# Druthyn/rtiow

Measured on AMD Instinct MI355X. Metric: Msamples/sec (pixels×spp) on book-1 final scene; per-pixel RMSE vs CPU, higher is better.
Workload: dtype f64

## Files before the change

__graft_entry__.py:

```python
import os
import subprocess
import sys

ROOT = os.path.dirname(os.path.abspath(__file__))
if ROOT not in sys.path:
    sys.path.insert(0, ROOT)

HIPCC_FLAGS = [
    "-O3", "-std=c++17", "--offload-arch=gfx950",
    "-ffp-contract=off",
    "-fhip-fp32-correctly-rounded-divide-sqrt",
    "-mllvm", "-amdgpu-mfma-vgpr-form",
    "-fPIC", "-shared",
]


def build_hip_library(crosscheck=False, count_features=False):
    out = os.path.join(ROOT, "tools", "librtiow_hip_xcheck.so") if crosscheck else os.path.join(ROOT, "rtiow_amd", "librtiow_hip.so")
    if count_features:
        out = os.path.join(ROOT, "tools", "lib_features_count.so")
    srcs = [os.path.join(ROOT, "rtiow_amd", "csrc", name) for name in ("rt_api.hip", "rt_frames.hip", "rt_features.hip")]
    import bench
    cmd = ["hipcc", *HIPCC_FLAGS, *(["-DRTIOW_CROSSCHECK_MODES"] if crosscheck else []), *(["-DRT_FEATURES_COUNT"] if count_features else []),
           f'-DRT_SOURCE_SHA="{bench.kernel_source_sha()}"',
           "-I", os.path.join(ROOT, "include"), "-I", os.path.join(ROOT, "rtiow_amd", "csrc"), "-o", out, *srcs]
    subprocess.run(cmd, check=True, cwd=ROOT)
    return out


def build_host_cli(sanitize=False):
    out = os.path.join(ROOT, "host", "rtiow_render_san" if sanitize else "rtiow_render")
    rocm = os.environ.get("ROCM_PATH", "/opt/rocm")
    opt = ["-O1", "-g", "-fno-omit-frame-pointer", "-fsanitize=address,undefined", "-fno-sanitize-recover=all"] if sanitize else ["-O2"]
    cmd = ["g++", *opt, "-std=c++17", "-ffp-contract=off", "-Wall", "-Wextra", "-Wno-unused-parameter",
           "-I", os.path.join(ROOT, "include"), "-I", os.path.join(ROOT, "host"), "-isystem", os.path.join(rocm, "include"),
           "-o", out, os.path.join(ROOT, "host", "rtiow_render.cpp"),
           "-L", os.path.join(ROOT, "rtiow_amd"), "-lrtiow_hip", "-L", os.path.join(rocm, "lib"), "-lamdhip64", "-lrccl",
           "-pthread", "-Wl,-rpath,$ORIGIN/../rtiow_amd", "-Wl,-rpath," + os.path.join(rocm, "lib")]
    subprocess.run(cmd, check=True, cwd=ROOT)
    return out


def build() -> None:
    build_hip_library()
    build_hip_library(crosscheck=True)
    build_host_cli()
    subprocess.run(["make", "-s", "-C", os.path.join(ROOT, "oracle"), "liboracle.so"], check=True)
    import rtiow_amd
    from rtiow_amd import _ffi
    lib = _ffi.load()
    assert lib.rt_backend_name() == b"hip-gfx950"
    assert not _ffi.has_crosscheck_modes()
    assert rtiow_amd.SPHERE_DTYPE.itemsize == 72


def smoke() -> None:
    import numpy as np
    import oracle
    import rtiow_amd as rt

    w, h, spp = 96, 54, 4
    flat = rt.random_scene(1).flatten()
    cam = rt.book1_camera(w, h)
    with rt.Renderer(0) as r:
        r.upload_scene(flat)
        sums, fix, st = r.render(cam, rt.make_params(w, h, spp, seed=1))
        rgba = r.resolve_rgba8(fix, spp, flip=True)
    want_fix, want_sum, ost = oracle.render_b(oracle.camera_from_host(cam), flat, oracle.make_params(w, h, spp, seed=1))
    assert np.array_equal(fix, want_fix), "GPU exact sums differ from the CPU oracle"
    assert np.array_equal(sums, want_sum)
    assert st["rays_traced"] == ost["rays_traced"] and st["samples"] == w * h * spp
    assert np.array_equal(rgba, oracle.resolve_b(want_fix, spp, flip=True))
    with rt.Renderer(0) as r:
        r.upload_scene(flat)
# ... 11 lines not shown
```

rtiow_amd/_ffi.py:

```python
import ctypes as C
import os

_HERE = os.path.dirname(os.path.abspath(__file__))
LIB_PATH = os.environ.get("RTIOW_HIP_LIB") or os.path.join(_HERE, "librtiow_hip.so")


class rt_sphere(C.Structure):
    _fields_ = [("center", C.c_double * 3), ("radius", C.c_double), ("albedo", C.c_double * 3),
                ("param", C.c_double), ("kind", C.c_int32), ("reserved", C.c_int32)]


class rt_camera(C.Structure):
    _fields_ = [("origin", C.c_double * 3), ("lower_left_corner", C.c_double * 3),
                ("horizontal", C.c_double * 3), ("vertical", C.c_double * 3),
                ("u", C.c_double * 3), ("v", C.c_double * 3), ("lens_radius", C.c_double)]


class rt_params(C.Structure):
    _fields_ = [("width", C.c_int32), ("height", C.c_int32), ("spp", C.c_int32),
                ("sample_begin", C.c_int32), ("max_depth", C.c_int32), ("t_min", C.c_double),
                ("seed", C.c_uint64), ("tile_rows", C.c_int32), ("shard_index", C.c_int32),
                ("shard_count", C.c_int32), ("flags", C.c_uint32)]


# ... 13 lines not shown
RT_FLAG_DIAG_STATS = 0x4
RT_FLAG_UNIFORM53 = 0x8
RT_FLAG_OVERLAPPED = 0x10
RT_FLAG_KNOWN = 0x1f
RT_FEATURE_WORDS = 8

_VP = C.c_void_p
SYMBOLS = [
    ("rt_create", C.c_int, [C.c_int32, C.POINTER(_VP)]),
    ("rt_destroy", C.c_int, [_VP]),
    ("rt_upload_scene", C.c_int, [_VP, C.POINTER(rt_sphere), C.c_int32]),
    ("rt_shard_rows", C.c_int, [C.POINTER(rt_params), C.POINTER(C.c_int32)]),
    ("rt_shard_row_index", C.c_int, [C.POINTER(rt_params), C.c_int32, C.POINTER(C.c_int32)]),
    ("rt_render", C.c_int, [_VP, C.POINTER(rt_camera), C.POINTER(rt_params), _VP, _VP, C.POINTER(rt_stats)]),
    ("rt_render_device", C.c_int, [_VP, C.POINTER(rt_camera), C.POINTER(rt_params), _VP, _VP]),
    ("rt_fix_to_f32_device", C.c_int, [_VP, _VP, C.c_int64, _VP, _VP]),
    ("rt_last_stats", C.c_int, [_VP, C.POINTER(rt_stats)]),
    ("rt_resolve_rgba8_device", C.c_int, [_VP, _VP, C.c_int32, C.c_int32, C.c_int64, C.c_int32, _VP, _VP]),
    ("rt_resolve_rgba8", C.c_int, [_VP, _VP, C.c_int32, C.c_int32, C.c_int64, C.c_int32, _VP]),
    ("rt_render_rgba8", C.c_int, [_VP, C.POINTER(rt_camera), C.POINTER(rt_params), C.c_int32, _VP, C.POINTER(rt_stats)]),
    ("rt_render_pixels_device", C.c_int, [_VP, C.POINTER(rt_camera), C.POINTER(rt_params), _VP, C.c_int64, _VP, _VP]),
    ("rt_render_pixels", C.c_int, [_VP, C.POINTER(rt_camera), C.POINTER(rt_params), _VP, C.c_int64, _VP, C.POINTER(rt_stats)]),
    ("rt_select_pixels_device", C.c_int, [_VP, _VP, _VP, _VP, C.c_int32, C.c_int32, C.c_int32, C.POINTER(rt_adaptive), _VP, _VP, _VP]),
    ("rt_select_pixels_host", C.c_int, [_VP, _VP, _VP, C.c_int32, C.c_int32, C.c_int32, C.POINTER(rt_adaptive), _VP, C.POINTER(C.c_int64)]),
    ("rt_render_adaptive", C.c_int, [_VP, C.POINTER(rt_camera), C.POINTER(rt_params), C.POINTER(rt_adaptive), _VP, _VP, _VP, C.POINTER(rt_stats)]),
    ("rt_resolve_rgba8_counts_device", C.c_int, [_VP, _VP, _VP, C.c_int32, C.c_int32, C.c_int32, _VP, _VP]),
    ("rt_resolve_rgba8_counts", C.c_int, [_VP, _VP, _VP, C.c_int32, C.c_int32, C.c_int32, _VP]),
    ("rt_render_frames_device", C.c_int, [_VP, _VP, C.c_int32, C.c_int32, C.POINTER(rt_params), _VP, _VP]),
    ("rt_render_frames", C.c_int, [_VP, _VP, C.c_int32, C.c_int32, C.POINTER(rt_params), _VP, C.POINTER(rt_stats)]),
    ("rt_render_frames_rgba8", C.c_int, [_VP, _VP, C.c_int32, C.c_int32, C.POINTER(rt_params), C.c_int32, _VP, C.POINTER(rt_stats)]),
    ("rt_render_features_device", C.c_int, [_VP, C.POINTER(rt_camera), C.POINTER(rt_params), _VP, _VP, _VP]),
    ("rt_render_features", C.c_int, [_VP, C.POINTER(rt_camera), C.POINTER(rt_params), _VP, _VP, C.POINTER(C.c_float)]),
    ("rt_features_to_f32_device", C.c_int, [_VP, _VP, C.c_int32, C.c_int32, C.c_int64, _VP, _VP]),
    ("rt_features_to_f32", C.c_int, [_VP, _VP, C.c_int32, C.c_int32, C.c_int64, _VP]),
    ("rt_last_error", C.c_char_p, []),
    ("rt_backend_name", C.c_char_p, []),
    ("rt_abi_version", C.c_int32, []),
    ("rt_build_source_sha", C.c_char_p, []),
    ("rt_philox_device", C.c_int, [_VP, C.POINTER(C.c_uint32), C.POINTER(C.c_uint32), C.POINTER(C.c_uint32)]),
    ("rt_f64_div_sqrt_device", C.c_int, [_VP, _VP, _VP, C.c_int32, _VP, _VP]),
    ("rt_quantize_device", C.c_int, [_VP, _VP, C.c_int32, _VP]),
    ("rt_unit_accept_device", C.c_int, [_VP, _VP, C.c_int32, _VP, _VP]),
    ("rt_tube_tile_host", C.c_int, [C.POINTER(rt_sphere), _VP, _VP, C.POINTER(C.c_float)]),
    ("rt_tile_layout_host", C.c_int, [C.POINTER(rt_sphere), C.c_int32, C.POINTER(C.c_int32), C.POINTER(C.c_float), C.POINTER(C.c_int32), C.c_int32]),
    ("rt_filter_tube_device", C.c_int, [_VP, _VP, _VP, C.POINTER(rt_sphere), _VP, _VP, _VP, C.POINTER(C.c_float)]),
]

XCHECK_SYMBOLS = [
    ("rt_filter_products_device", C.c_int, [_VP, _VP, _VP, _VP, C.c_int32, _VP, _VP]),
    ("rt_filter_lifted_device", C.c_int, [_VP, _VP, _VP, C.POINTER(rt_sphere), _VP, _VP, _VP]),
    ("rt_grid_cells_device", C.c_int, [_VP, _VP, _VP, C.c_int32, C.POINTER(C.c_float), C.c_int32, C.c_float, _VP, _VP]),
]

_lib = None


class RtiowHipError(RuntimeError):
    pass


def load():
    global _lib
    if _lib is not None:
        return _lib
    if not os.path.exists(LIB_PATH):
        raise RtiowHipError(
            f"{LIB_PATH} not found: build it with ./build_lib.sh (hipcc --offload-arch=gfx950); "
            "there is no CPU fallback for the render path")
    try:
        import torch
    except ImportError:
        pass
    lib = C.CDLL(LIB_PATH)
    for name, res, args in SYMBOLS:
        fn = getattr(lib, name)
        fn.restype = res
        fn.argtypes = args
    for name, res, args in XCHECK_SYMBOLS:
        if hasattr(lib, name):
            fn = getattr(lib, name)
            fn.restype = res
            fn.argtypes = args
    _lib = lib
    return lib


def has_crosscheck_modes():
    return hasattr(load(), "rt_filter_lifted_device")


def check(rc, what):
    if rc != 0:
        msg = load().rt_last_error().decode("utf-8", "replace")
        raise RtiowHipError(f"{what} failed ({rc}): {msg}")
```

rtiow_amd/csrc/rt_api.hip:

```cpp
#include <hip/hip_runtime.h>

#include <algorithm>
#include <cmath>
#include <cstdarg>
#include <cstdio>
#include <cstdlib>
#include <cstring>
#include <vector>

#include "rt_host.hpp"

namespace {

thread_local char g_err[512] = "";

int env_int(const char *name, int dflt)
{
    const char *v = getenv(name);
    if (!v || !*v) return dflt;
    return atoi(v);
}

}

// ... 586 lines not shown
    const bool large_blocks = mode_now == 5 && !(p->flags & RT_FLAG_DIAG_STATS) && use_ring && small_block == (unsigned)rt::kItemBlock &&
                              p->spp >= (small_grid_scene ? rt::kLargeMinSppSmallGrid : rt::kLargeMinSpp) && total_items >= lb_min;
    const unsigned item_block = large_blocks ? rt::kItemBlockLarge : use_ring ? small_block : rt::kItemBlock;
    const unsigned long long n_blocks = (total_items + item_block - 1) / item_block;
    if (n_blocks > 0x7fffffffULL)
        return fail(RT_ERR_INVALID_ARGUMENT, "rows*width*spp = %llu pixel-samples in one launch: at most 2^31 blocks of %d "
                    "(split the samples over several launches with sample_begin and RT_FLAG_ACCUMULATE)", total_items, (int)item_block);
    rt::KParams kp;
    memset(&kp, 0, sizeof(kp));
    static_assert(sizeof(rt::KCamera) == sizeof(rt_camera), "camera layouts must match");
    memcpy(&kp.cam, cam, sizeof(rt_camera));
    kp.width = p->width; kp.height = p->height;
    kp.spp = p->spp; kp.sample_begin = p->sample_begin; kp.max_depth = p->max_depth;
    kp.t_min = p->t_min;
    kp.k0 = (uint32_t)p->seed; kp.k1 = (uint32_t)(p->seed >> 32);
    kp.tile_rows = p->tile_rows; kp.shard_index = p->shard_index; kp.shard_count = p->shard_count;
    kp.rows = rows; kp.n_spheres = ctx->n_spheres;
    kp.npix = (uint32_t)npix; kp.total_items = total_items; kp.n_blocks = (uint32_t)n_blocks;
    kp.inv_spp = p->spp > 0 ? 1.0 / (double)p->spp : 0.0;
    kp.inv_width = 1.0 / (double)p->width;
    auto magic_for = [](long long d) -> uint32_t {
        return (d <= 1 || d >= 32768) ? 0u : (uint32_t)(0x100000000ULL / (unsigned long long)d + 1ULL);
    };
    kp.magic_spp = magic_for(p->spp); kp.magic_width = magic_for(p->width); kp.magic_tile = magic_for(p->tile_rows);
    kp.use_ring = use_ring ? 1 : 0;
    kp.block_items = item_block;
    set_scene_params(ctx, kp);
    kp.fix = (unsigned long long *)d_fix;
    rc = next_launch_slot(ctx, stream, kp);
    if (rc) return rc;

    if (!(p->flags & RT_FLAG_ACCUMULATE) && npix > 0)
        RT_HIP(hipMemsetAsync(d_fix, 0, (size_t)npix * 3 * sizeof(unsigned long long), stream));
    RT_HIP(hipMemsetAsync(ctx->d_queue, 0, 64, stream));
    RT_HIP(hipMemsetAsync(ctx->d_stats, 0, 1024, stream));

    memset(&ctx->last, 0, sizeof(ctx->last));
    ctx->last.n_spheres = ctx->n_spheres;
    ctx->last.block_threads = rt::kBlock;
    ctx->zero_depth_samples = 0;
    if (p->max_depth == 0 || kp.total_items == 0) {
        RT_HIP(hipEventRecord(ctx->ev0, stream));
        RT_HIP(hipEventRecord(ctx->ev1, stream));
        ctx->zero_depth_samples = (unsigned long long)npix * (unsigned long long)p->spp;
        ctx->launched = true;
        return RT_OK;
    }

    int grid = 0;
    const bool diag = (p->flags & RT_FLAG_DIAG_STATS) != 0;
    const int mode = (p->flags & RT_FLAG_NO_FILTER) ? 0 : ctx->scan_mode;
    ctx->last.scan_mode = mode;
    ctx->last.kernel_variant = 0;
    const bool small_grid = small_grid_scene;
    if (p->flags & RT_FLAG_UNIFORM53) {
        if (diag || (mode != 0 && mode != 5))
            return fail(RT_ERR_INVALID_ARGUMENT, "RT_FLAG_UNIFORM53 runs with scan mode 5 (the default) or RT_FLAG_NO_FILTER, without RT_FLAG_DIAG_STATS");
        if (mode == 0) rc = launch_render<0, false, false, true>(ctx, kp, stream, &grid);
        else if (small_grid) rc = large_blocks ? launch_render<5, false, true, true, rt::kItemBlockLarge>(ctx, kp, stream, &grid)
                                              : launch_render<5, false, true, true>(ctx, kp, stream, &grid);
        else rc = large_blocks ? launch_render<5, false, false, true, rt::kItemBlockLarge>(ctx, kp, stream, &grid)
                               : launch_render<5, false, false, true>(ctx, kp, stream, &grid);
        if (rc) return rc;
        ctx->last.kernel_variant = 2 | ((mode == 5 && small_grid) ? 1 : 0) | (mode == 5 && large_blocks ? 4 : 0);
        ctx->launched = true;
        ctx->last.grid_blocks = grid;
        return RT_OK;
    }
    switch (mode * 2 + (diag ? 1 : 0)) {
    case 0: rc = launch_render<0, false>(ctx, kp, stream, &grid); break;
    case 1: rc = launch_render<0, true>(ctx, kp, stream, &grid); break;
    case 2: rc = launch_render<1, false>(ctx, kp, stream, &grid); break;
    case 3: rc = launch_render<1, true>(ctx, kp, stream, &grid); break;
#ifdef RTIOW_CROSSCHECK_MODES
    case 4: rc = launch_render<2, false>(ctx, kp, stream, &grid); break;
    case 5: rc = launch_render<2, true>(ctx, kp, stream, &grid); break;
    case 6: rc = launch_render<3, false>(ctx, kp, stream, &grid); break;
    case 7: rc = launch_render<3, true>(ctx, kp, stream, &grid); break;
    case 8: rc = launch_render<4, false>(ctx, kp, stream, &grid); break;
    case 9: rc = launch_render<4, true>(ctx, kp, stream, &grid); break;
#endif
    case 10:
        if (small_grid) {
            rc = large_blocks ? launch_render<5, false, true, false, rt::kItemBlockLarge>(ctx, kp, stream, &grid)
                              : launch_render<5, false, true>(ctx, kp, stream, &grid);
            ctx->last.kernel_variant = 1;
        } else rc = large_blocks ? launch_render<5, false, false, false, rt::kItemBlockLarge>(ctx, kp, stream, &grid)
                                 : launch_render<5, false>(ctx, kp, stream, &grid);
        if (large_blocks) ctx->last.kernel_variant |= 4;
        break;
    default: rc = launch_render<5, true>(ctx, kp, stream, &grid); break;
    }
    if (rc) return rc;
    ctx->launched = true;
    ctx->last.grid_blocks = grid;
    return RT_OK;
}

int rt_last_stats(rt_context *ctx, rt_stats *stats)
{
    if (!ctx || !stats) return fail(RT_ERR_INVALID_ARGUMENT, "ctx/stats is NULL");
    if (!ctx->launched) return fail(RT_ERR_INVALID_ARGUMENT, "no launch to report on");
    RT_HIP(hipSetDevice(ctx->device));
    RT_HIP(hipEventSynchronize(ctx->ev1));
    float ms = 0.0f;
    RT_HIP(hipEventElapsedTime(&ms, ctx->ev0, ctx->ev1));
    unsigned long long h[80];
    RT_HIP(hipMemcpy(h, ctx->d_stats, sizeof(h), hipMemcpyDeviceToHost));
    for (int k = 0; k < 64; ++k) ctx->last.live_per_bounce[k] = h[16 + k];
    ctx->last.rays_traced = h[0];
    ctx->last.samples = h[1] + ctx->zero_depth_samples;
    ctx->last.candidates = h[2];
    ctx->last.exact_roots = h[3];
    ctx->last.direct_samples = h[4];
    ctx->last.sphere_tests = h[0] * (unsigned long long)(ctx->last.n_spheres > 0 ? ctx->last.n_spheres : 0);
    ctx->last.kernel_ms = ms;
    *stats = ctx->last;
    return RT_OK;
}

#if defined(RT_PHASE_STAMPS) || defined(RT_BLOCK_COUNTS) || defined(RT_EXIT_TIMES) || defined(RT_LDS_CONFLICTS)
extern "C" int rt_debug_phase_cycles(rt_context *ctx, unsigned long long out[8])
{
    RT_HIP(hipSetDevice(ctx->device));
    RT_HIP(hipEventSynchronize(ctx->ev1));
    RT_HIP(hipMemcpy(out, ctx->d_stats + 8, 64, hipMemcpyDeviceToHost));
    return RT_OK;
}
extern "C" int rt_debug_phase_cycles16(rt_context *ctx, unsigned long long out[16])
{
    RT_HIP(hipSetDevice(ctx->device));
    RT_HIP(hipEventSynchronize(ctx->ev1));
    RT_HIP(hipMemcpy(out, ctx->d_stats + 8, 64, hipMemcpyDeviceToHost));
    RT_HIP(hipMemcpy(out + 8, ctx->d_stats + 80, 64, hipMemcpyDeviceToHost));
    return RT_OK;
// ... 545 lines not shown
```

rtiow_amd/csrc/rt_diag.hpp:

```cpp
#pragma once
#include <hip/hip_runtime.h>
#include <stdint.h>

#if (defined(RT_PHASE_STAMPS) + defined(RT_BLOCK_COUNTS) + defined(RT_EXIT_TIMES) + defined(RT_LDS_CONFLICTS)) > 1
#error "one diagnostic build at a time: RT_PHASE_STAMPS, RT_BLOCK_COUNTS, RT_EXIT_TIMES or RT_LDS_CONFLICTS"
#endif

#define RT_DIAG_NOTHING do { } while (0)

#define RT_DIAG_DECLARE() RT_DIAG_NOTHING
#define RT_DIAG_FLUSH() RT_DIAG_NOTHING
#define RT_STAMP(k) RT_DIAG_NOTHING
#define RT_COUNT(k) RT_DIAG_NOTHING
#define RT_COUNT_N(k, n) RT_DIAG_NOTHING
#define RT_COUNT_MAIN(k) RT_DIAG_NOTHING
#define RT_COUNT_ROWS_TRIP(k) RT_DIAG_NOTHING
#define RT_COUNT_ENUM_TRIP(m) RT_DIAG_NOTHING
#define RT_COUNT_REDRAW_LANES(ok) RT_DIAG_NOTHING
#define RT_LDS(site, BYTES, ATOMIC, LOAD64, ptr, active) RT_DIAG_NOTHING
#define RT_LDS_N(site, n, BYTES, ATOMIC, LOAD64, byte_addr, active) RT_DIAG_NOTHING
#define RT_LDS_QUEUE_READS(take, entry) RT_DIAG_NOTHING
#define RT_LDS_POOL_TIE(has_root, r, key) RT_DIAG_NOTHING
#define RT_LDS_ENUM_READS(has, word, summary, seg0) RT_DIAG_NOTHING
#define RT_LDS_RING_ADDS(ringed, my_blk) RT_DIAG_NOTHING

#if defined(RT_PHASE_STAMPS)
#undef RT_DIAG_DECLARE
#undef RT_DIAG_FLUSH
#undef RT_STAMP
#define RT_DIAG_DECLARE() unsigned long long ph[16] = {0, 0, 0, 0, 0, 0, 0, 0, 0, 0, 0, 0, 0, 0, 0, 0}, tprev = __builtin_amdgcn_s_memtime()
#define RT_STAMP(k) do { __builtin_amdgcn_s_waitcnt(0); const unsigned long long tn_ = __builtin_amdgcn_s_memtime(); \
                         __builtin_amdgcn_s_waitcnt(0); ph[k] += tn_ - tprev; tprev = tn_; } while (0)
#define RT_DIAG_FLUSH() do { if (lane == 0) { \
        for (int k_ = 0; k_ < 8; ++k_) atomicAdd(P.stats + 8 + k_, ph[k_]); \
        for (int k_ = 8; k_ < 16; ++k_) atomicAdd(P.stats + 80 + (k_ - 8), ph[k_]); } } while (0)
#endif

#if defined(RT_EXIT_TIMES)
#undef RT_DIAG_DECLARE
#undef RT_DIAG_FLUSH
#define RT_DIAG_DECLARE() const unsigned long long t_wave_start = __builtin_amdgcn_s_memrealtime()
#define RT_DIAG_FLUSH() do { if (lane == 0) { \
        const unsigned long long te_ = __builtin_amdgcn_s_memrealtime(); \
        atomicMax(P.stats + 8, te_); atomicMax(P.stats + 9, ~te_); atomicAdd(P.stats + 10, te_); \
        atomicMax(P.stats + 11, ~t_wave_start); atomicAdd(P.stats + 12, 1ull); } } while (0)
#endif

#if defined(RT_BLOCK_COUNTS)
#undef RT_DIAG_DECLARE
#undef RT_DIAG_FLUSH
#undef RT_COUNT
#undef RT_COUNT_N
#define RT_DIAG_DECLARE() __shared__ unsigned int s_cnt[kBlock / 64][8]; if ((tid & 63) < 8) s_cnt[tid >> 6][tid & 7] = 0u
#define RT_COUNT(k) do { if ((int)(tid & 63) == (int)__builtin_ctzll(__ballot(true))) s_cnt[tid >> 6][k] += 1u; } while (0)
#define RT_COUNT_N(k, n) do { if ((int)(tid & 63) == (int)__builtin_ctzll(__ballot(true))) s_cnt[tid >> 6][k] += (unsigned)(n); } while (0)
#define RT_DIAG_FLUSH() do { if (lane == 0) for (int k_ = 0; k_ < 8; ++k_) atomicAdd(P.stats + 8 + k_, (unsigned long long)s_cnt[tid >> 6][k_]); } while (0)
#if defined(RT_COUNT_ROWS)
#undef RT_COUNT_ROWS_TRIP
#define RT_COUNT_ROWS_TRIP(k) RT_COUNT(k)
#elif defined(RT_COUNT_ENUM)
#undef RT_COUNT_ENUM_TRIP
#define RT_COUNT_ENUM_TRIP(m) do { RT_COUNT(1); RT_COUNT_N(6, __popcll(m)); } while (0)
#elif defined(RT_COUNT_REDRAW)
#undef RT_COUNT_REDRAW_LANES
#define RT_COUNT_REDRAW_LANES(ok) do { const unsigned n1_ = (unsigned)__popcll(__ballot(true)), n6_ = (unsigned)__popcll(__ballot(!(ok))); \
                                       RT_COUNT_N(1, n1_); RT_COUNT_N(6, n6_); } while (0)
#else
#undef RT_COUNT_MAIN
#define RT_COUNT_MAIN(k) RT_COUNT(k)
#endif
#endif

#if defined(RT_LDS_CONFLICTS)
namespace rt {
template <int BYTES, bool ATOMIC, bool LOAD64 = false>
__device__ __noinline__ uint32_t lds_extra_cycles(uint32_t byte_addr, bool active)
{
    constexpr int G = (BYTES == 8 && !LOAD64) ? 16 : 32;
    const int lane = threadIdx.x & 63;
    const unsigned long long m = __ballot(active);
    const uint32_t unit = byte_addr / (uint32_t)BYTES;
    const uint32_t bank = unit % (uint32_t)G;
    bool first = active;
    for (int k = 0; k < 64; ++k) {
        const uint32_t uk = (uint32_t)__builtin_amdgcn_readlane((int)unit, k);
        if (((m >> k) & 1ull) && k < lane && k / G == lane / G && uk == unit) first = false;
    }
    const unsigned long long counted = ATOMIC ? m : __ballot(first);
    uint32_t cnt = 0;
    for (int k = 0; k < 64; ++k) {
        const uint32_t bk = (uint32_t)__builtin_amdgcn_readlane((int)bank, k);
        if (((counted >> k) & 1ull) && k / G == lane / G && bk == bank) cnt++;
    }
    if (!active) cnt = 0;
    uint32_t extra = 0;
    for (int g = 0; g < 64 / G; ++g) {
        uint32_t mx = 0;
        for (int k = g * G; k < (g + 1) * G; ++k) mx = max(mx, (uint32_t)__builtin_amdgcn_readlane((int)cnt, k));
        extra += mx > 1u ? mx - 1u : 0u;
    }
    return extra;
}
}
#undef RT_DIAG_DECLARE
#undef RT_DIAG_FLUSH
#undef RT_LDS
#undef RT_LDS_N
#undef RT_LDS_QUEUE_READS
#undef RT_LDS_POOL_TIE
#undef RT_LDS_ENUM_READS
#undef RT_LDS_RING_ADDS
#define RT_DIAG_DECLARE() unsigned long long lds_x[8] = {0, 0, 0, 0, 0, 0, 0, 0}
#define RT_DIAG_FLUSH() do { if (lane == 0) for (int k_ = 0; k_ < 8; ++k_) atomicAdd(P.stats + 8 + k_, lds_x[k_]); } while (0)
#define RT_LDS(site, BYTES, ATOMIC, LOAD64, ptr, active) do { lds_x[site] += rt::lds_extra_cycles<BYTES, ATOMIC, LOAD64>( \
        (uint32_t)(uintptr_t)(const void __attribute__((address_space(3))) *)(ptr), (active)); } while (0)
#define RT_LDS_N(site, n, BYTES, ATOMIC, LOAD64, byte_addr, active) do { lds_x[site] += (unsigned long long)(n) * \
        rt::lds_extra_cycles<BYTES, ATOMIC, LOAD64>((uint32_t)(byte_addr), (active)); } while (0)
#define RT_LDS_QUEUE_READS(take, entry) do { const bool take_ = (take); const uint32_t e_ = take_ ? (entry) : 0u; \
        RT_LDS(6, 8, false, true, &quv_w[e_], take_); RT_LDS(6, 8, false, true, &quv_w[64 + e_], take_); \
// ... 12 lines not shown
```

rtiow_amd/csrc/rt_host.hpp:

```cpp
#pragma once
#include <hip/hip_runtime.h>

#include "rtiow_hip.h"
#include "rt_kernels.hpp"
#ifdef RTIOW_CROSSCHECK_MODES
#include "xcheck/rt_xcheck_host_ctx.hpp"
#endif

namespace rt_host {
int fail(int code, const char *fmt, ...);
}

#define RT_HIP(call)                                                                          \
    do {                                                                                      \
        hipError_t e_ = (call);                                                               \
        if (e_ != hipSuccess)                                                                 \
            return rt_host::fail(e_ == hipErrorOutOfMemory ? RT_ERR_OUT_OF_MEMORY : RT_ERR_HIP,        \
                        "%s failed: %s (%s:%d)", #call, hipGetErrorString(e_), __FILE__, __LINE__); \
    } while (0)

struct rt_context {
    int device = 0;
    int cu_count = 0;
    float *d_filt = nullptr;
    double *d_geo = nullptr;
    double *d_mat = nullptr;
    uint4 *d_btube = nullptr;
    float tube_rho = 1.0f;
    double *d_geo_slot = nullptr;
    uint32_t *d_slot_orig = nullptr;
    int n_global = 0;
    int grid_dim = 0;
    float grid[8] = {};
    float scene_scale = 0.0f;
#ifdef RTIOW_CROSSCHECK_MODES
    XcheckScene x;
#endif
    int n_tiles = 0;
    int n_always = 0;
    int always_idx[8] = {0, 0, 0, 0, 0, 0, 0, 0};
    int scan_mode = 5;
    int n_spheres = -1;
    static constexpr int kSlots = 2;
    unsigned int *q_slots[kSlots] = {nullptr, nullptr};
    unsigned long long *s_slots[kSlots] = {nullptr, nullptr};
    hipEvent_t e0_slots[kSlots] = {nullptr, nullptr}, e1_slots[kSlots] = {nullptr, nullptr};
    bool slot_used[kSlots] = {false, false};
    int cur = 0;
    unsigned int *d_queue = nullptr;
    unsigned long long *d_stats = nullptr;
    hipEvent_t ev0 = nullptr, ev1 = nullptr;
    hipStream_t own_stream = nullptr;
    bool launched = false;
    unsigned long long zero_depth_samples = 0;
    rt_stats last{};
    void *d_stage_fix = nullptr; size_t stage_fix_bytes = 0;
    void *d_stage_sum = nullptr; size_t stage_sum_bytes = 0;
    void *d_stage_rgba = nullptr; size_t stage_rgba_bytes = 0;
    int blocks_per_cu = 0;
    void *d_sel = nullptr; size_t sel_bytes = 0;
    void *d_adapt = nullptr; size_t adapt_bytes = 0;
    void *d_stage_list = nullptr; size_t stage_list_bytes = 0;
    void *d_stage_cams = nullptr; size_t stage_cams_bytes = 0;
    int ring_min_spp = 0;
};

namespace rt_host {

int validate_params(const rt_params *p);
int ensure(void **ptr, size_t *have, size_t need);
void set_scene_params(const rt_context *ctx, rt::KParams &kp);
int next_launch_slot(rt_context *ctx, hipStream_t stream, rt::KParams &kp);

template <int MODE, bool DIAG, bool SMALLGRID = false, bool U53 = false, int ITEMS = rt::kItemBlock>
int launch_render(rt_context *ctx, const rt::KParams &kp, hipStream_t stream, int *grid_out)
{
    int per_cu = ctx->blocks_per_cu;
    if (per_cu <= 0) {
        int occ = 0;
        RT_HIP(hipOccupancyMaxActiveBlocksPerMultiprocessor(&occ, rt::render_kernel<MODE, DIAG, SMALLGRID, U53, ITEMS>, rt::kBlock, 0));
        per_cu = occ < 1 ? 1 : (occ > 8 ? 8 : occ);
    }
    long long grid = (long long)ctx->cu_count * per_cu;
    const long long need = (long long)((kp.total_items + rt::kBlock - 1) / rt::kBlock);
    if (grid > need) grid = need;
    if (grid < 1) grid = 1;
    *grid_out = (int)grid;
    RT_HIP(hipEventRecord(ctx->ev0, stream));
    hipLaunchKernelGGL((rt::render_kernel<MODE, DIAG, SMALLGRID, U53, ITEMS>), dim3((unsigned)grid), dim3(rt::kBlock), 0, stream, kp);
    RT_HIP(hipGetLastError());
    RT_HIP(hipEventRecord(ctx->ev1, stream));
    return RT_OK;
}

}
```

rtiow_amd/csrc/rt_kernels.hpp:

```cpp
#pragma once
#include "rt_device.hpp"
#include "rt_diag.hpp"
#ifdef RTIOW_CROSSCHECK_MODES
#include "xcheck/rt_xcheck_params.hpp"
#endif
#include <type_traits>

#ifndef RT_GROUP_SKIP
#define RT_GROUP_SKIP 1
#endif

namespace rt {

struct KCamera {
    double origin[3], llc[3], horizontal[3], vertical[3], u[3], v[3];
    double lens_radius;
};

struct KParams {
    KCamera cam;
    double t_min;
    int32_t width, height;
    int32_t spp, sample_begin, max_depth;
    uint32_t k0, k1;
    int32_t tile_rows, shard_index, shard_count;
    int32_t rows;
    int32_t n_spheres;
    int32_t use_ring;
    uint32_t npix;
    uint32_t n_blocks;
    unsigned long long total_items;
    double inv_spp;
    double inv_width;
    uint32_t magic_spp, magic_width, magic_tile;
    uint32_t block_items;
    const float *filt;
#ifdef RTIOW_CROSSCHECK_MODES
    KXcheckTables x;
#endif
    const uint4 *btube;
    float tube_rho;
    float scene_scale;
    const double *geo_slot;
    const uint32_t *slot_orig;
    float grid[8];
    int32_t grid_dim;
    unsigned long long grid_rows;
    int32_t n_global;
    int32_t n_tiles;
    int32_t n_always;
    int32_t always_idx[8];
    const double *geo;
    const double *mat;
    unsigned long long *fix;
    unsigned int *queue;
    unsigned long long *stats;
    const uint32_t *pix_list;
    const KCamera *cams;
    unsigned long long frame_items;
    double inv_frame_blocks;
    uint32_t frame_blocks;
    uint32_t frame_pix;
    int32_t sample_stride;
};

constexpr int RT_KIND_LAMBERTIAN = 0, RT_KIND_METAL = 1, RT_KIND_DIALECTRIC = 2;
constexpr int kBlock = 256;
constexpr int kCandCap = 24;
constexpr int kScanUnroll = 8;
constexpr int kItemBlock = 256;
constexpr int kItemBlockLarge = 1024;
constexpr int kItemBlockList = -kItemBlock;
constexpr int kItemBlockFrames = -2 * kItemBlock;
static_assert(kItemBlockLarge + 32768 < 65536, "udiv_small: numerators x < d + kItemBlockLarge with d < 2^15 keep x * d < 2^32");
constexpr int kLargeMinSpp = 147;
constexpr int kLargeMinSppSmallGrid = 69;
constexpr unsigned long long kLargeMinItems = 200000000ull;
constexpr int kRingSlots = 8;
constexpr int kRingDepth = 4;
constexpr int kMatStride = 10;
constexpr int kListCap = 126;
constexpr int kSegTilesTube = 28;
constexpr int kSegTiles = 36;

__device__ __forceinline__ D3 ld3(const double *p) { return mk(p[0], p[1], p[2]); }

__device__ __forceinline__ uint32_t udiv_small(uint32_t x, uint32_t d, uint32_t magic)
{
    const uint32_t big = x >= d ? 1u : 0u;
    const uint32_t q = __umulhi(x, magic);
    return d == 1u ? x : (d >= 32768u ? big : q);
}



constexpr int kRowPad = 80;

typedef float f32x4 __attribute__((ext_vector_type(4)));

template <int MODE, bool DIAG, bool SMALLGRID = false, bool U53 = false, int ITEMS = 256>
__global__ __launch_bounds__(kBlock, (MODE == 5 && !DIAG) ? 4 : (MODE >= 2) ? 3 : 5) void render_kernel(const KParams P)
{
    constexpr bool PIXLIST = ITEMS == kItemBlockList;
    constexpr bool FRAMES = ITEMS == kItemBlockFrames;
    static_assert(ITEMS > 0 || PIXLIST || FRAMES, "ITEMS: a block size, kItemBlockList or kItemBlockFrames");
    static_assert(!(PIXLIST || FRAMES) || (MODE == 5 && !DIAG && !U53), "pixel lists and frame batches: the shipped kernel, 32-bit uniforms, blocks of 256");
    constexpr bool kWideRing = SMALLGRID || (MODE == 5 && !DIAG && (ITEMS == kItemBlock || ITEMS == kItemBlockList || ITEMS == kItemBlockFrames));
    constexpr int kRingDepth = kWideRing ? 2 : 4;
    constexpr int kRingSlots = kWideRing ? 16 : 8;
    static_assert(kRingDepth * kRingSlots == rt::kRingDepth * rt::kRingSlots, "same LDS either way");
    __shared__ uint16_t cand[MODE == 1 ? kCandCap : 1][MODE == 1 ? kBlock : 1];
    constexpr bool MATRIX = (MODE >= 2);
    constexpr bool LIFTED = (MODE == 4);
    constexpr bool TUBE = (MODE == 5);
    constexpr bool RAYOP = (MODE == 2 || MODE == 3);
    __shared__ float s_rayop[RAYOP ? kBlock / 64 : 1][RAYOP ? 8 : 1][RAYOP ? kRowPad : 1];
    constexpr int kSeg = TUBE ? kSegTilesTube : kSegTiles;
    static_assert(TUBE || (kSeg / 2) * 64 * sizeof(unsigned int) >= 32 * kStageStride * sizeof(uint4), "operand staging fits the bitmap");
    static_assert(!TUBE || ((kSeg / 2) * 64 + kListCap + 2) * sizeof(unsigned int) == 64 * 4 * sizeof(uint4), "tube: staging = bitmap + tile list");
    constexpr int kBitWords = TUBE ? (kSeg / 2) * 64 + kListCap + 2 : (kSeg / 2) * 64;
    __shared__ __attribute__((aligned(16))) unsigned int s_bits[MATRIX ? kBlock / 64 : 1][MATRIX ? kBitWords : 1];
    __shared__ unsigned int s_sum[(MATRIX && !TUBE) ? kBlock : 1];
    __shared__ double s_quv[kBlock / 64][2][64];
    __shared__ unsigned int s_qid[kBlock / 64][5][64];
    __shared__ unsigned int s_pool[MATRIX ? kBlock / 64 : 1][MATRIX ? 128 : 1];
    __shared__ unsigned long long s_best[MATRIX ? kBlock : 1];
    __shared__ unsigned int s_bidx[MATRIX ? kBlock : 1];
    __shared__ unsigned long long s_ring[kBlock / 64][kRingDepth][kRingSlots * 3];
    __shared__ unsigned int s_rpix[kBlock / 64][kRingDepth];
    __shared__ unsigned int s_live[DIAG ? kBlock / 64 : 1][DIAG ? 64 : 1];
    __shared__ double s_thr[3][kBlock];

    const int tid = threadIdx.x;
    const int lane = tid & 63;
    {
        unsigned long long *z = &s_ring[tid >> 6][0][0];
        for (int k = lane; k < kRingDepth * kRingSlots * 3; k += 64) z[k] = 0ull;
        if (lane < kRingDepth) s_rpix[tid >> 6][lane] = 0u;
    }
    if (DIAG) s_live[tid >> 6][tid & 63] = 0u;
    auto rank_below = [](unsigned long long m) -> uint32_t {
        return __builtin_amdgcn_mbcnt_hi((uint32_t)(m >> 32), __builtin_amdgcn_mbcnt_lo((uint32_t)m, 0u));
    };

    const float __attribute__((address_space(4))) *filt =
        (const float __attribute__((address_space(4))) *)(uintptr_t)P.filt;
    const double *__restrict__ geo = P.geo;
    const double *__restrict__ mat = P.mat;
    const int n = P.n_spheres;
    const double t_min = P.t_min;
    const double wm1 = (double)(P.width - 1);
    const double hm1 = (double)(P.height - 1);

    bool dead = false, alive = false;
    uint32_t pix_local = 0, pix_global = 0;
    int s = 0;
    uint32_t my_frame = 0;
    uint32_t my_blk = 0;
    D3 o = mk(0, 0, 0), d = mk(0, 0, 1);
    int depth = 0;
// ... 631 lines not shown
                finish_pool();
                __builtin_amdgcn_s_setprio(0);
                }
            }
#ifdef RTIOW_CROSSCHECK_MODES
#include "xcheck/rt_xcheck_scan.inc"
#endif
        }
        RT_STAMP(2);
        if (alive && !MATRIX) {
            if (MODE == 0) {
                for (int i = 0; i < n; ++i) { if (DIAG) n_cand++; exact_test(i, std::true_type{}); }
            } else {
                const RayFilter f = make_filter(o, d);
                int cnt = 0;
                auto drain = [&]() { test_list(cnt); cnt = 0; };
                auto test = [&](float cx, float cy, float cz, float kp, int i) {
                    const bool keep = filter_keeps(f, cx, cy, cz, kp);
                    if (__builtin_expect(__ballot(keep) != 0ull, 0)) {
                        if (keep) {
                            cand[cnt][tid] = (uint16_t)i;
                            cnt++;
                        }
                    }
                };
                constexpr int BW = 4 * kScanUnroll;
                const int nb = n / kScanUnroll;
                for (int bidx = 0; bidx < nb; ++bidx) {
                    const float __attribute__((address_space(4))) *q = filt + (size_t)BW * (size_t)bidx;
                    float rec[BW];
#pragma unroll
                    for (int k = 0; k < BW; ++k) rec[k] = q[k];
#pragma unroll
                    for (int k = 0; k < kScanUnroll; ++k)
                        test(rec[4 * k + 0], rec[4 * k + 1], rec[4 * k + 2], rec[4 * k + 3], bidx * kScanUnroll + k);
                    if (__any(cnt > kCandCap - kScanUnroll)) drain();
                }
                for (int i = nb * kScanUnroll; i < n; ++i) {
                    const float __attribute__((address_space(4))) *q = filt + 4 * (size_t)i;
                    test(q[0], q[1], q[2], q[3], i);
                }
                drain();
            }
        }

        if (DIAG) {
            unsigned long long pk = (unsigned long long)n_cand | ((unsigned long long)n_roots << 32);
#pragma unroll
            for (int sh = 32; sh >= 1; sh >>= 1) pk += __shfl_xor(pk, sh);
            tot_cand += pk & 0xFFFFFFFFull; tot_roots += pk >> 32;
        }
        RT_STAMP(3);
        bool finished = false;
        D3 radiance = mk(0.0, 0.0, 0.0);
        if (alive) {
            bool done = false;
            D3 L = mk(0.0, 0.0, 0.0);
            const bool is_hit = hit >= 0;
            int kind = -1;
            bool front = false;
            D3 p = o, nrm = mk(0.0, 0.0, 0.0), sp = mk(0.0, 0.0, 0.0), albedo = mk(1.0, 1.0, 1.0);
            double param = 0.0, inv_param = 0.0, r0_front = 0.0, r0_back = 0.0;
            uint32_t w_first = 0u, w_second = 0u;
            if (is_hit) {
                const double *mrec = mat + kMatStride * (size_t)hit;
                const double4 g = *reinterpret_cast<const double4 *>(geo + 4 * (size_t)hit);
                const double2 mA = *reinterpret_cast<const double2 *>(mrec);
                const double2 mB = *reinterpret_cast<const double2 *>(mrec + 2);
                const double2 mC = *reinterpret_cast<const double2 *>(mrec + 4);
                const double2 mD_ = *reinterpret_cast<const double2 *>(mrec + 6);
                const double2 mE_ = *reinterpret_cast<const double2 *>(mrec + 8);
                U4 w = philox4x32_10(pix_global, (uint32_t)s, ev, 0u, P.k0, P.k1);
                asm volatile("" : "+v"(w.x), "+v"(w.y), "+v"(w.z), "+v"(w.w));
                kind = (int)mC.y;
                param = mA.y;
                albedo = mk(mB.x, mB.y, mC.x);
                p = o + d * closest;
                const D3 outward = (p - mk(g.x, g.y, g.z)) * mA.x;
                front = dot(d, outward) < 0.0;
                nrm = front ? outward : (mk(0.0, 0.0, 0.0) - outward);
                w_first = w.x;
                if constexpr (U53) w_second = w.y;
                RT_STAMP(11);
                if constexpr (U53) {
                  if (kind != RT_KIND_DIALECTRIC) {
                    U4 b1 = philox4x32_10(pix_global, (uint32_t)s, ev + 1u, 0u, P.k0, P.k1);
                    uint32_t nblk = 2u, c0 = b1.z, c1 = b1.w;
                    double sx = u11_53(w.x, w.y), sy = u11_53(w.z, w.w), sz = u11_53(b1.x, b1.y);
                    bool ok = sx * sx + sy * sy + sz * sz < 1.0;
                    while (!ok) {
                        RT_COUNT_MAIN(6);
                        U4 b = philox4x32_10(pix_global, (uint32_t)s, ev + nblk, 0u, P.k0, P.k1);
                        nblk++;
                        sx = u11_53(c0, c1); sy = u11_53(b.x, b.y); sz = u11_53(b.z, b.w);
                        ok = sx * sx + sy * sy + sz * sz < 1.0;
                        if (!ok) {
                            b = philox4x32_10(pix_global, (uint32_t)s, ev + nblk, 0u, P.k0, P.k1);
                            b1 = philox4x32_10(pix_global, (uint32_t)s, ev + nblk + 1u, 0u, P.k0, P.k1);
                            nblk += 2u;
                            sx = u11_53(b.x, b.y); sy = u11_53(b.z, b.w); sz = u11_53(b1.x, b1.y);
                            c0 = b1.z; c1 = b1.w;
                            ok = sx * sx + sy * sy + sz * sz < 1.0;
                        }
                    }
                    ev += nblk;
                    sp = mk(sx, sy, sz);
                  } else {
                    inv_param = mD_.x; r0_front = mD_.y; r0_back = mE_.x;
                  }
                } else
                if (kind != RT_KIND_DIALECTRIC) {
                    uint32_t tx = w.x, ty = w.y, tz = w.z, nblk = 1u;
                    bool ok = unit_sphere_accepts(tx, ty, tz);
                    RT_COUNT_REDRAW_LANES(ok);
                    if (!ok) {
                        uint32_t c0 = w.w;
                        do {
                            RT_COUNT_MAIN(6);
                            U4 b = philox4x32_10(pix_global, (uint32_t)s, ev + nblk, 0u, P.k0, P.k1);
                            nblk++;
                            tx = c0; ty = b.x; tz = b.y;
                            ok = unit_sphere_accepts(tx, ty, tz);
                            if (!ok) {
                                const uint32_t c1 = b.z, c2 = b.w;
                                b = philox4x32_10(pix_global, (uint32_t)s, ev + nblk, 0u, P.k0, P.k1);
                                nblk++;
                                tx = c1; ty = c2; tz = b.x;
                                ok = unit_sphere_accepts(tx, ty, tz);
                                if (!ok) {
                                    tx = b.y; ty = b.z; tz = b.w;
                                    ok = unit_sphere_accepts(tx, ty, tz);
                                    if (!ok) {
                                        b = philox4x32_10(pix_global, (uint32_t)s, ev + nblk, 0u, P.k0, P.k1);
                                        nblk++;
                                        tx = b.x; ty = b.y; tz = b.z; c0 = b.w;
                                        ok = unit_sphere_accepts(tx, ty, tz);
                                    }
                                }
                            }
                        } while (!ok);
                    }
                    ev += nblk;
                    sp = mk(u11(tx), u11(ty), u11(tz));
                } else {
                    inv_param = mD_.x; r0_front = mD_.y; r0_back = mE_.x;
                }
            }
            RT_STAMP(12);
            D3 V = d;
            if (kind == RT_KIND_LAMBERTIAN) V = sp;
            if (kind == RT_KIND_METAL) V = reflect(d, nrm);
            const D3 uV = unit_vector(V);
            if (!is_hit) {
                const double t = 0.5 * (uV.y + 1.0);
                const D3 sky = mk(1.0, 1.0, 1.0) * (1.0 - t) + mk(0.5, 0.7, 1.0) * t;
                L = mk(s_thr[0][tid], s_thr[1][tid], s_thr[2][tid]) * sky;
                done = true;
            } else {
                D3 ndir;
                if (kind == RT_KIND_LAMBERTIAN) {
                    ndir = nrm + uV;
                    const double eps = 1e-8;
                    const bool near_zero = __builtin_fabs(ndir.x) < eps && __builtin_fabs(ndir.y) < eps && __builtin_fabs(ndir.z) < eps;
                    if (__builtin_expect(__ballot(near_zero) != 0ull, 0)) {
                        if (near_zero) ndir = nrm;
                    }
                } else if (kind == RT_KIND_METAL) {
                    ndir = uV + sp * param;
                    if (dot(ndir, nrm) <= 0.0) done = true;
                } else {
                    const double ratio = front ? inv_param : param;
                    const double cos_theta = min_1(-dot(uV, nrm));
                    const double sin_theta = __builtin_sqrt(1.0 - cos_theta * cos_theta);
                    bool do_refract = false;
                    if (ratio * sin_theta <= 1.0) {
                        const double r0 = front ? r0_front : r0_back;
                        const double x = 1.0 - cos_theta;
                        const double x2 = x * x;
                        const double refl = r0 + (1.0 - r0) * ((x2 * x2) * x);
                        ev++;
                        do_refract = refl <= (U53 ? u01_53(w_first, w_second) : u01(w_first));
                    }
                    ndir = do_refract ? refract(uV, nrm, ratio) : reflect(uV, nrm);
                }
                if (kind != RT_KIND_DIALECTRIC) {
                    s_thr[0][tid] = s_thr[0][tid] * albedo.x;
                    s_thr[1][tid] = s_thr[1][tid] * albedo.y;
                    s_thr[2][tid] = s_thr[2][tid] * albedo.z;
                }
                o = p;
                d = ndir;
                depth -= 1;
                if (depth <= 0) done = true;
            }
            if (done) {
                alive = false;
                finished = true;
                radiance = L;
            }
        }
        RT_STAMP(13);
        __builtin_amdgcn_s_setprio(1);
        {
            const uint32_t age = (blk_seq - (my_blk >> 4)) & 0x0FFFFFFFu;
            const bool direct = finished && !(P.use_ring && age < (uint32_t)kRingDepth);
            const bool ringed = finished && !direct;
            RT_LDS_RING_ADDS(ringed, my_blk);
            if (finished) {
                const unsigned long long q0 = quantize(radiance.x), q1 = quantize(radiance.y), q2 = quantize(radiance.z);
                if (ringed) {
                    unsigned long long *acc = ring_w + ((my_blk >> 4) & (uint32_t)(kRingDepth - 1)) * (kRingSlots * 3) + (my_blk & 15u) * 3u;
                    atomicAdd(acc + 0, q0); atomicAdd(acc + 1, q1); atomicAdd(acc + 2, q2);
                } else {
                    unsigned long long *px = P.fix + (size_t)pix_local * 3u;
                    atomicAdd(px + 0, q0); atomicAdd(px + 1, q1); atomicAdd(px + 2, q2);
                }
            }
            n_direct += (uint32_t)__popcll(__ballot(direct));
            unsigned long long fm = __ballot(ringed);
            if (fm != 0ull) {
                __builtin_amdgcn_wave_barrier();
                const unsigned long long m0 = __ballot(ringed && age == 0u);
                rem0 -= (uint32_t)__popcll(m0);
                if (m0 != 0ull && rem0 == 0u) flush_ring(blk_seq & (uint32_t)(kRingDepth - 1));
                fm &= ~m0;
                if constexpr (kRingDepth == 2) {
                    if (fm != 0ull) {
                        rem1 -= (uint32_t)__popcll(fm);
                        if (rem1 == 0u) flush_ring((blk_seq - 1u) & 1u);
                    }
                } else
                if (fm != 0ull) {
                    const unsigned long long m1 = __ballot(ringed && age == 1u);
                    rem1 -= (uint32_t)__popcll(m1);
                    if (m1 != 0ull && rem1 == 0u) flush_ring((blk_seq - 1u) & 3u);
                    fm &= ~m1;
                    if (fm != 0ull) {
                        const unsigned long long m2 = __ballot(ringed && age == 2u);
                        rem2 -= (uint32_t)__popcll(m2);
                        if (m2 != 0ull && rem2 == 0u) flush_ring((blk_seq - 2u) & 3u);
                        fm &= ~m2;
                        if (fm != 0ull) {
                            rem3 -= (uint32_t)__popcll(fm);
                            if (rem3 == 0u) flush_ring((blk_seq - 3u) & 3u);
                        }
                    }
                }
            }
        }
        n_samples += (uint32_t)__popcll(__ballot(finished));
        RT_STAMP(4);
    }
// ... 272 lines not shown
```

Measured before the change: 8297.

## Add capped rejection-sampling kernel variant that parks rays after fixed redraw tries

```diff
diff --git a/__graft_entry__.py b/__graft_entry__.py
--- a/__graft_entry__.py
+++ b/__graft_entry__.py
@@ -19,7 +19,7 @@
     out = os.path.join(ROOT, "tools", "librtiow_hip_xcheck.so") if crosscheck else os.path.join(ROOT, "rtiow_amd", "librtiow_hip.so")
     if count_features:
         out = os.path.join(ROOT, "tools", "lib_features_count.so")
-    srcs = [os.path.join(ROOT, "rtiow_amd", "csrc", name) for name in ("rt_api.hip", "rt_frames.hip", "rt_features.hip")]
+    srcs = [os.path.join(ROOT, "rtiow_amd", "csrc", name) for name in ("rt_api.hip", "rt_frames.hip", "rt_features.hip", "rt_dense.hip")]
     import bench
     cmd = ["hipcc", *HIPCC_FLAGS, *(["-DRTIOW_CROSSCHECK_MODES"] if crosscheck else []), *(["-DRT_FEATURES_COUNT"] if count_features else []),
            f'-DRT_SOURCE_SHA="{bench.kernel_source_sha()}"',
diff --git a/include/rtiow_hip_diag.h b/include/rtiow_hip_diag.h
--- /dev/null
+++ b/include/rtiow_hip_diag.h
@@ -0,0 +1,16 @@
+#ifndef RTIOW_HIP_DIAG_H
+#define RTIOW_HIP_DIAG_H
+
+#include "rtiow_hip.h"
+
+#ifdef __cplusplus
+extern "C" {
+#endif
+
+int32_t rt_last_dense_body(const rt_context *ctx);
+
+#ifdef __cplusplus
+}
+#endif
+
+#endif
diff --git a/rtiow_amd/_ffi.py b/rtiow_amd/_ffi.py
--- a/rtiow_amd/_ffi.py
+++ b/rtiow_amd/_ffi.py
@@ -89,6 +89,10 @@
     ("rt_grid_cells_device", C.c_int, [_VP, _VP, _VP, C.c_int32, C.POINTER(C.c_float), C.c_int32, C.c_float, _VP, _VP]),
 ]
 
+DIAG_SYMBOLS = [
+    ("rt_last_dense_body", C.c_int32, [_VP]),
+]
+
 _lib = None
 
 
@@ -113,6 +117,10 @@
         fn = getattr(lib, name)
         fn.restype = res
         fn.argtypes = args
+    for name, res, args in DIAG_SYMBOLS:
+        fn = getattr(lib, name)
+        fn.restype = res
+        fn.argtypes = args
     for name, res, args in XCHECK_SYMBOLS:
         if hasattr(lib, name):
             fn = getattr(lib, name)
diff --git a/rtiow_amd/csrc/rt_api.hip b/rtiow_amd/csrc/rt_api.hip
--- a/rtiow_amd/csrc/rt_api.hip
+++ b/rtiow_amd/csrc/rt_api.hip
@@ -662,6 +662,7 @@
     const int mode = (p->flags & RT_FLAG_NO_FILTER) ? 0 : ctx->scan_mode;
     ctx->last.scan_mode = mode;
     ctx->last.kernel_variant = 0;
+    ctx->last_dense_body = 0;
     const bool small_grid = small_grid_scene;
     if (p->flags & RT_FLAG_UNIFORM53) {
         if (diag || (mode != 0 && mode != 5))
@@ -691,6 +692,12 @@
     case 9: rc = launch_render<4, true>(ctx, kp, stream, &grid); break;
 #endif
     case 10:
+        if (dense_body_is_capped(small_grid, large_blocks)) {
+            rc = launch_dense_capped(ctx, kp, stream, small_grid, large_blocks, &grid);
+            ctx->last.kernel_variant = (small_grid ? 1 : 0) | (large_blocks ? 4 : 0);
+            ctx->last_dense_body = 1;
+            break;
+        }
         if (small_grid) {
             rc = large_blocks ? launch_render<5, false, true, false, rt::kItemBlockLarge>(ctx, kp, stream, &grid)
                               : launch_render<5, false, true>(ctx, kp, stream, &grid);
diff --git a/rtiow_amd/csrc/rt_dense.hip b/rtiow_amd/csrc/rt_dense.hip
--- /dev/null
+++ b/rtiow_amd/csrc/rt_dense.hip
@@ -0,0 +1,39 @@
+#include <hip/hip_runtime.h>
+
+#include <cstdlib>
+#include <cstring>
+
+#define RT_RENDER_KERNEL_ONLY
+#include "rt_host.hpp"
+#include "rtiow_hip_diag.h"
+
+namespace rt_host {
+
+static bool capped_by_default(bool small_grid, bool large_blocks)
+{
+    return kDenseCappedDefault[small_grid ? 1 : 0][large_blocks ? 1 : 0];
+}
+
+bool dense_body_is_capped(bool small_grid, bool large_blocks)
+{
+    const char *v = getenv("RTIOW_DENSE_BODY");
+    if (v && !strcmp(v, "classic")) return false;
+    if (v && !strcmp(v, "capped")) return true;
+    return capped_by_default(small_grid, large_blocks);
+}
+
+int launch_dense_capped(rt_context *ctx, const rt::KParams &kp, hipStream_t stream, bool small_grid, bool large_blocks, int *grid_out)
+{
+    if (small_grid)
+        return large_blocks ? launch_render<5, false, true, false, rt::kItemBlockDenseLarge>(ctx, kp, stream, grid_out)
+                            : launch_render<5, false, true, false, rt::kItemBlockDense>(ctx, kp, stream, grid_out);
+    return large_blocks ? launch_render<5, false, false, false, rt::kItemBlockDenseLarge>(ctx, kp, stream, grid_out)
+                        : launch_render<5, false, false, false, rt::kItemBlockDense>(ctx, kp, stream, grid_out);
+}
+
+}
+
+extern "C" int32_t rt_last_dense_body(const rt_context *ctx)
+{
+    return ctx ? ctx->last_dense_body : -1;
+}
diff --git a/rtiow_amd/csrc/rt_diag.hpp b/rtiow_amd/csrc/rt_diag.hpp
--- a/rtiow_amd/csrc/rt_diag.hpp
+++ b/rtiow_amd/csrc/rt_diag.hpp
@@ -17,6 +17,7 @@
 #define RT_COUNT_ROWS_TRIP(k) RT_DIAG_NOTHING
 #define RT_COUNT_ENUM_TRIP(m) RT_DIAG_NOTHING
 #define RT_COUNT_REDRAW_LANES(ok) RT_DIAG_NOTHING
+#define RT_COUNT_CAPPED_PARKS(n) RT_DIAG_NOTHING
 #define RT_LDS(site, BYTES, ATOMIC, LOAD64, ptr, active) RT_DIAG_NOTHING
 #define RT_LDS_N(site, n, BYTES, ATOMIC, LOAD64, byte_addr, active) RT_DIAG_NOTHING
 #define RT_LDS_QUEUE_READS(take, entry) RT_DIAG_NOTHING
@@ -65,6 +66,11 @@
 #undef RT_COUNT_REDRAW_LANES
 #define RT_COUNT_REDRAW_LANES(ok) do { const unsigned n1_ = (unsigned)__popcll(__ballot(true)), n6_ = (unsigned)__popcll(__ballot(!(ok))); \
                                        RT_COUNT_N(1, n1_); RT_COUNT_N(6, n6_); } while (0)
+#elif defined(RT_COUNT_PARKS)
+#undef RT_COUNT_CAPPED_PARKS
+#undef RT_COUNT_MAIN
+#define RT_COUNT_CAPPED_PARKS(n) RT_COUNT_N(1, n)
+#define RT_COUNT_MAIN(k) do { if ((k) == 6) RT_COUNT(k); } while (0)
 #else
 #undef RT_COUNT_MAIN
 #define RT_COUNT_MAIN(k) RT_COUNT(k)
diff --git a/rtiow_amd/csrc/rt_host.hpp b/rtiow_amd/csrc/rt_host.hpp
--- a/rtiow_amd/csrc/rt_host.hpp
+++ b/rtiow_amd/csrc/rt_host.hpp
@@ -62,6 +62,7 @@
     void *d_adapt = nullptr; size_t adapt_bytes = 0;
     void *d_stage_list = nullptr; size_t stage_list_bytes = 0;
     void *d_stage_cams = nullptr; size_t stage_cams_bytes = 0;
+    int last_dense_body = 0;
     int ring_min_spp = 0;
 };
 
@@ -93,4 +94,8 @@
     return RT_OK;
 }
 
+constexpr bool kDenseCappedDefault[2][2] = {{false, false}, {false, true}};
+bool dense_body_is_capped(bool small_grid, bool large_blocks);
+int launch_dense_capped(rt_context *ctx, const rt::KParams &kp, hipStream_t stream, bool small_grid, bool large_blocks, int *grid_out);
+
 }
diff --git a/rtiow_amd/csrc/rt_kernels.hpp b/rtiow_amd/csrc/rt_kernels.hpp
--- a/rtiow_amd/csrc/rt_kernels.hpp
+++ b/rtiow_amd/csrc/rt_kernels.hpp
@@ -72,6 +72,8 @@
 constexpr int kItemBlockLarge = 1024;
 constexpr int kItemBlockList = -kItemBlock;
 constexpr int kItemBlockFrames = -2 * kItemBlock;
+constexpr int kItemBlockDense = -3 * kItemBlock;
+constexpr int kItemBlockDenseLarge = -4 * kItemBlock;
 static_assert(kItemBlockLarge + 32768 < 65536, "udiv_small: numerators x < d + kItemBlockLarge with d < 2^15 keep x * d < 2^32");
 constexpr int kLargeMinSpp = 147;
 constexpr int kLargeMinSppSmallGrid = 69;
@@ -103,9 +105,11 @@
 {
     constexpr bool PIXLIST = ITEMS == kItemBlockList;
     constexpr bool FRAMES = ITEMS == kItemBlockFrames;
-    static_assert(ITEMS > 0 || PIXLIST || FRAMES, "ITEMS: a block size, kItemBlockList or kItemBlockFrames");
+    constexpr bool CAPPED = ITEMS == kItemBlockDense || ITEMS == kItemBlockDenseLarge;
+    static_assert(ITEMS > 0 || PIXLIST || FRAMES || CAPPED, "ITEMS: a block size, kItemBlockList, kItemBlockFrames, kItemBlockDense or kItemBlockDenseLarge");
     static_assert(!(PIXLIST || FRAMES) || (MODE == 5 && !DIAG && !U53), "pixel lists and frame batches: the shipped kernel, 32-bit uniforms, blocks of 256");
-    constexpr bool kWideRing = SMALLGRID || (MODE == 5 && !DIAG && (ITEMS == kItemBlock || ITEMS == kItemBlockList || ITEMS == kItemBlockFrames));
+    static_assert(!CAPPED || (MODE == 5 && !DIAG && !U53), "the capped redraw: the shipped kernel, 32-bit uniforms (a 53-bit try is six words: another period)");
+    constexpr bool kWideRing = SMALLGRID || (MODE == 5 && !DIAG && (ITEMS == kItemBlock || ITEMS == kItemBlockList || ITEMS == kItemBlockFrames || ITEMS == kItemBlockDense));
     constexpr int kRingDepth = kWideRing ? 2 : 4;
     constexpr int kRingSlots = kWideRing ? 16 : 8;
     static_assert(kRingDepth * kRingSlots == rt::kRingDepth * rt::kRingSlots, "same LDS either way");
@@ -843,6 +847,7 @@
         }
         RT_STAMP(3);
         bool finished = false;
+        bool parked = false;
         D3 radiance = mk(0.0, 0.0, 0.0);
         if (alive) {
             bool done = false;
@@ -899,6 +904,36 @@
                   } else {
                     inv_param = mD_.x; r0_front = mD_.y; r0_back = mE_.x;
                   }
+                } else if constexpr (CAPPED) {
+                  if (kind != RT_KIND_DIALECTRIC) {
+                    uint32_t tx = w.x, ty = w.y, tz = w.z, nblk = 1u;
+                    bool ok = unit_sphere_accepts(tx, ty, tz);
+                    RT_COUNT_REDRAW_LANES(ok);
+                    if (!ok) {
+                        RT_COUNT_MAIN(6);
+                        U4 b = philox4x32_10(pix_global, (uint32_t)s, ev + 1u, 0u, P.k0, P.k1);
+                        nblk = 2u;
+                        tx = w.w; ty = b.x; tz = b.y;
+                        ok = unit_sphere_accepts(tx, ty, tz);
+                        if (!ok) {
+                            RT_COUNT_MAIN(6);
+                            const uint32_t c1 = b.z, c2 = b.w;
+                            b = philox4x32_10(pix_global, (uint32_t)s, ev + 2u, 0u, P.k0, P.k1);
+                            nblk = 3u;
+                            tx = c1; ty = c2; tz = b.x;
+                            ok = unit_sphere_accepts(tx, ty, tz);
+                            if (!ok) {
+                                tx = b.y; ty = b.z; tz = b.w;
+                                ok = unit_sphere_accepts(tx, ty, tz);
+                            }
+                        }
+                    }
+                    parked = !ok;
+                    ev += nblk;
+                    sp = mk(u11(tx), u11(ty), u11(tz));
+                  } else {
+                    inv_param = mD_.x; r0_front = mD_.y; r0_back = mE_.x;
+                  }
                 } else
                 if (kind != RT_KIND_DIALECTRIC) {
                     uint32_t tx = w.x, ty = w.y, tz = w.z, nblk = 1u;
@@ -974,6 +1009,20 @@
                     }
                     ndir = do_refract ? refract(uV, nrm, ratio) : reflect(uV, nrm);
                 }
+                if constexpr (CAPPED) {
+                    if (parked) done = false;
+                    else {
+                        if (kind != RT_KIND_DIALECTRIC) {
+                            s_thr[0][tid] = s_thr[0][tid] * albedo.x;
+                            s_thr[1][tid] = s_thr[1][tid] * albedo.y;
+                            s_thr[2][tid] = s_thr[2][tid] * albedo.z;
+                        }
+                        o = p;
+                        d = ndir;
+                        depth -= 1;
+                        if (depth <= 0) done = true;
+                    }
+                } else {
                 if (kind != RT_KIND_DIALECTRIC) {
                     s_thr[0][tid] = s_thr[0][tid] * albedo.x;
                     s_thr[1][tid] = s_thr[1][tid] * albedo.y;
@@ -983,12 +1032,18 @@
                 d = ndir;
                 depth -= 1;
                 if (depth <= 0) done = true;
+                }
             }
             if (done) {
                 alive = false;
                 finished = true;
                 radiance = L;
             }
+        }
+        if constexpr (CAPPED) {
+            const uint32_t n_parked = (uint32_t)__popcll(__ballot(parked));
+            RT_COUNT_CAPPED_PARKS(n_parked);
+            n_rays -= n_parked;
         }
         RT_STAMP(13);
         __builtin_amdgcn_s_setprio(1);
```

Result: faster. 8397, median of 6 (+1.2%).
